# laomao0/BIN

Hardware: AMD Instinct MI355X
Metric: interpolated frames/sec at 1280x720 (higher is better)
Workload: dtype f16x3 (fp16 hi+lo pairs = 22-bit significands, 3 MFMA products, f32 accumulate; fp32-class: 1e-6 vs the fp32 reference); 1 GPU; Adobe240 test_blur 1280x720 inference, batch=1 per GPU (6-frame window padded to 768x1344 by the test.py rule), window-sharded; precision=f16x3, streams=1, pipelined_steps=False, four_call_schedule=False, parity=max-abs <= 2e-5 (f16x3) vs the fp32 reference (tests/)

## Files before the change

### bin_amd/_lib.py

```python
import ctypes as C
import os

from .build import GRAD_LIB_PATH, LIB_PATH, OPT_LIB_PATH

RDN_LAYERS = 66
RDN_MAX_LAYERS, RDN_MAX_CONVS = 192, 7
PLAN_KEEP_ACTS, PLAN_NO_FUSE, PLAN_RDB3, PLAN_FUSED_UPNET, PLAN_FUSED_UPNET_TRAIN = 1, 2, 4, 8, 16
BWD_ACCUMULATE = 1
BWD_SAVED_X3 = 2
BWD_FUSED_UPNET = 4
EPI_PLANES, EPI_SHUFFLE, EPI_FINAL, EPI_FINAL_SUBPIX = 0, 1, 2, 4
PROF_WGRAD = 16
LOSS_CHARBONNIER, LOSS_L1_SUM, LOSS_L2_SUM = 0, 1, 2
RDN_LAYOUT_WORDS, RDN_BWD_LAYOUT_WORDS = 16, 24


class BinConvDesc(C.Structure):
    _fields_ = [("N", C.c_int32), ("H", C.c_int32), ("W", C.c_int32), ("ksize", C.c_int32),
                ("cin_chunks", C.c_int32), ("cout", C.c_int32), ("cout_pad", C.c_int32),
                ("nterms", C.c_int32), ("epilogue", C.c_int32), ("relu", C.c_int32),
                ("x_cpg", C.c_int32), ("x_group_stride", C.c_int64), ("n_images", C.c_int32),
                ("reserved", C.c_int32), ("status", C.c_void_p)]


LOSS_MAX_TERMS = 24
CONV_HALF_LAST_CHUNK = 1


class BinLossTerms(C.Structure):
    _fields_ = [("x", C.c_void_p * LOSS_MAX_TERMS), ("y", C.c_void_p * LOSS_MAX_TERMS), ("n_terms", C.c_int32)]


class BinLossGrads(C.Structure):
    _fields_ = [("out", C.c_void_p * LOSS_MAX_TERMS), ("term_a", C.c_int32 * LOSS_MAX_TERMS),
                ("term_b", C.c_int32 * LOSS_MAX_TERMS), ("sign_a", C.c_float * LOSS_MAX_TERMS),
                ("sign_b", C.c_float * LOSS_MAX_TERMS), ("n_out", C.c_int32)]


class BinRdnShape(C.Structure):
    _fields_ = [("G0", C.c_int32), ("D", C.c_int32), ("C", C.c_int32), ("G", C.c_int32)]

# ... 235 lines not shown
```

### bin_amd/csrc/binhip_conv.hip

```cpp
#include "binhip_conv_common.h"
#include <vector>
#include <cstdio>
#include <cstdlib>

template <int KS, int MT, int WM, int R, int WN, int KC, int NT, int NBUF, int EPI>
struct ConvCfg {
    static constexpr int PAD = KS / 2;
    static constexpr int COUTB = 32 * MT * WM;
    static constexpr int TH = R * WN;
    static constexpr int PH = TH + KS - 1;
    static constexpr int PW = 32 + KS - 1;
    static constexpr int PP = (PH * PW * 2 + 63) / 64;
    static constexpr int WP = KS * KS * MT * WM;
    static constexpr int CHUNK_BYTES = (PP + WP) * 1024;
    static constexpr int NPL = (NT == 3) ? 2 : 1;
    static constexpr int PLANE_BYTES = KC * CHUNK_BYTES;
    static constexpr int BUF_BYTES = NPL * PLANE_BYTES;
    static constexpr int NW = WM * WN;
    static constexpr int LDS_BYTES = NBUF * BUF_BYTES + 1024;
    static constexpr int NPJ = (PP + NW - 1) / NW;
    static constexpr int NWJ = (WP + NW - 1) / NW;
    static constexpr int PS = NPL * KC * (NPJ + NWJ);
    static_assert(NW == 4 || NW == 8 || NW == 16, "4, 8 or 16 waves per workgroup");
    static_assert(LDS_BYTES <= 160 * 1024, "LDS budget");
// ... 229 lines not shown
    if (ksize == 3 && nterms == 3) return 32;
    if (ksize == 3 && cout_pad == 256) return 128;
    if (ksize == 5) return 32;
    if (ksize == 1 && cout_pad == 224) return 224;
    if (ksize == 1 && cout_pad == 1152) return 192;
    if (cout_pad % 96 == 0) return 96;
    if (ksize == 3 && cout_pad % 64 == 0) return 64;
    return 32;
}

static int bh_dispatch_conv(const ConvKArgs& a, int k, int cp, int nt, int e, hipStream_t s);
int bh_launch_conv_x3(const ConvKArgs& a, int cout_pad, int epilogue, hipStream_t s);
int bh_launch_final_dot2(const ConvKArgs& a, hipStream_t s);
int bh_launch_conv_x3_k5(const ConvKArgs& a, int cout_pad, hipStream_t s);
int bh_launch_conv_x3_k5_subpix(const ConvKArgs& a, hipStream_t s);
int bh_launch_final_m16(const ConvKArgs& a, hipStream_t s);

int bh_prepare_conv(const BhConvCall& c, ConvKArgs* out) {
    const BinConvDesc& d = c.d;
    if (!c.x_hi || !c.w_hi || !c.bias) return BINHIP_E_ARG;
    if (d.nterms != 1 && d.nterms != 3) return BINHIP_E_ARG;
    if (d.nterms == 3 && (!c.x_lo || !c.w_lo)) return BINHIP_E_ARG;
    if (d.N <= 0 || d.H <= 0 || d.W <= 0 || d.cin_chunks <= 0) return BINHIP_E_SHAPE;
    if ((long long)d.N * d.H * d.W >= (1ll << 26)) return BINHIP_E_SHAPE;
    ConvKArgs a;
    a.x_hi = (const _Float16*)c.x_hi; a.x_lo = (const _Float16*)c.x_lo;
    a.w_hi = (const _Float16*)c.w_hi; a.w_lo = (const _Float16*)c.w_lo;
    a.bias = c.bias;
    a.y_hi = (_Float16*)c.y_hi; a.y_lo = (_Float16*)c.y_lo;
    a.r_hi = (const _Float16*)c.r_hi; a.r_lo = (const _Float16*)c.r_lo;
    a.r2_hi = (const _Float16*)c.r2_hi; a.r2_lo = (const _Float16*)c.r2_lo;
    a.m_hi = (const _Float16*)c.m_hi;
    a.flags = (unsigned*)c.status;
    a.res_chunks = c.res_chunks > 0 ? c.res_chunks : (1 << 30);
    a.mask_from = c.mask_from;
    a.y_cpg = c.y_cpg; a.y_group_stride = c.y_group_stride;
    a.y_cpg_inv = c.y_cpg > 0 ? (unsigned)(((1u << 20) + c.y_cpg - 1) / c.y_cpg) : 0u;
    if (c.y_cpg > 128 || (c.y_cpg > 0 && d.cout_pad / 16 >= 4096)) return BINHIP_E_SHAPE;
    a.half_last = (d.reserved & BINHIP_CONV_HALF_LAST_CHUNK) ? 1 : 0;
    a.y_unshuf = c.y_unshuf;
    if (c.y_unshuf && (d.epilogue != BINHIP_EPI_PLANES || c.y_cpg > 0 || (d.H & 1) || (d.W & 1) || c.y_unshuf * 16 < d.cout))
        return BINHIP_E_SHAPE;
    if (c.r2_hi && d.nterms == 3 && !c.r2_lo) return BINHIP_E_ARG;
    a.out_f32 = c.y_f32;
    for (int i = 0; i < 5; ++i) a.img[i] = c.images[i];
    a.group_stride = d.x_group_stride;
    a.N = d.N; a.H = d.H; a.W = d.W;
    a.nchunks = d.cin_chunks;
    a.cpg = d.x_cpg;
    a.relu = d.relu; a.has_res = (c.r_hi != nullptr); a.nimg = d.n_images; a.cout = d.cout;
    a.och_limit = (d.epilogue == BINHIP_EPI_PLANES) ? (d.cout + 15) / 16 : (1 << 30);
    a.tiles_x = a.tiles_y = 0;
    a.ncol = 1;
    a.xcd_remap = 1;
    a.dbg = 0;
// ... 44 lines not shown
    const BinConvDesc& d = c.d;
    const int k = d.ksize, cp = d.cout_pad, nt = d.nterms, e = d.epilogue;
    if (bh_prof_begin(c.prof, k, cp, e, s)) {
        const int rc = bh_dispatch_conv(a, k, cp, nt, e, s);
        bh_prof_end(c.prof, s);
        return rc;
    }
    return bh_dispatch_conv(a, k, cp, nt, e, s);
}

static int bh_dispatch_conv(const ConvKArgs& a, int k, int cp, int nt, int e, hipStream_t s) {
    const int P = BINHIP_EPI_PLANES, S = BINHIP_EPI_SHUFFLE, F = BINHIP_EPI_FINAL;
    const int cb = bh_conv_cout_block(k, cp, nt);
    if (cb <= 0 || cp % cb) return BINHIP_E_SHAPE;
    if (e == BINHIP_EPI_FINAL_SUBPIX)
        return nt == 3 ? bh_launch_conv_x3_k5_subpix(a, s) : launch_cfg<5, 1, 1, 2, 8, 1, 1, 2, BINHIP_EPI_FINAL_SUBPIX>(a, cp, s);
    if (e == F && k == 3 && cp == 32 && a.cout <= 3 && nt == 1)
        return bh_launch_final_dot2(a, s);
    if (e == F && k == 3 && cp == 32 && a.cout <= 3 && nt == 3 && a.nchunks <= 4)
        return bh_launch_final_m16(a, s);
    if (nt == 1) {
        if (e == F && k == 3 && cp == 32) return launch_cfg<3, 1, 1, 2, 8, 1, 1, 2, F>(a, cp, s);
        if (e == S && k == 3 && cp == 256) return launch_cfg<3, 2, 2, 4, 4, 1, 1, 2, S>(a, cp, s);
        if (e == P && k == 3 && cb == 32)  return launch_cfg<3, 1, 1, 2, 8, 1, 1, 2, P>(a, cp, s);
        if (e == P && k == 3 && cb == 64)  return launch_cfg<3, 2, 1, 2, 4, 1, 1, 2, P>(a, cp, s);
        if (e == P && k == 3 && cb == 96)  return launch_cfg<3, 3, 1, 2, 4, 1, 1, 2, P>(a, cp, s);
        if (e == P && k == 3 && cb == 128) return launch_cfg<3, 2, 2, 4, 4, 1, 1, 2, P>(a, cp, s);
        if (e == P && k == 1 && cb == 224) return launch_cfg<1, 7, 1, 1, 8, 2, 1, 2, P>(a, cp, s);
        if (e == P && k == 1 && cb == 192) return launch_cfg<1, 6, 1, 1, 8, 2, 1, 2, P>(a, cp, s);
        if (e == P && k == 1 && cb == 32)  return launch_cfg<1, 1, 1, 4, 4, 4, 1, 2, P>(a, cp, s);
        if (e == P && k == 1 && cb == 96) {
// ... 346 lines not shown
    if (shuffle_perm && (cout % 4 || cout != cout_pad)) return BINHIP_E_SHAPE;
    const long long total = (long long)cout_pad * cin_chunks * ksize * ksize * 2;
    const int th = 256;
    const long long nb = (total + th - 1) / th;
    hipLaunchKernelGGL(relayout_kernel, dim3((unsigned)nb), dim3(th), 0, (hipStream_t)stream, w_oihw, bias, cout, cin,
                       ksize, cout_pad, cin_chunks, cout_block, shuffle_perm, (_Float16*)w_hi, (_Float16*)w_lo,
                       bias_out);
    BH_CHECK_LAUNCH();
    return 0;
}

int binhip_conv2d_fwd(const BinConvDesc* d, const void* x_hi, const void* x_lo, const void* w_hi,
                      const void* w_lo, const float* bias, const void* res_hi, const void* res_lo,
                      void* y_hi, void* y_lo, float* y_f32, const float* const* images, void* stream) {
    if (!d) return BINHIP_E_ARG;
    if (d->reserved & ~BINHIP_CONV_HALF_LAST_CHUNK) return BINHIP_E_ARG;
    if ((d->reserved & BINHIP_CONV_HALF_LAST_CHUNK) && d->ksize != 5) return BINHIP_E_ARG;
    BhConvCall c;
    c.d = *d;
    c.x_hi = x_hi; c.x_lo = x_lo; c.w_hi = w_hi; c.w_lo = w_lo; c.bias = bias;
    c.r_hi = res_hi; c.r_lo = res_lo; c.y_hi = y_hi; c.y_lo = y_lo; c.y_f32 = y_f32;
    c.status = d->status;
    for (int i = 0; i < 5; ++i) c.images[i] = (images && i < d->n_images) ? images[i] : nullptr;
    if (d->epilogue == BINHIP_EPI_FINAL && d->n_images > 0 && !images) return BINHIP_E_ARG;
    return bh_launch_conv(c, (hipStream_t)stream);
}

}
```

### bin_amd/csrc/binhip_conv_common.h

```cpp
#pragma once
#include "binhip_internal.h"
#ifndef BINHIP_TIMELINE
#define BINHIP_TIMELINE 0
#endif

typedef _Float16 half8 __attribute__((ext_vector_type(8)));
typedef _Float16 half4 __attribute__((ext_vector_type(4)));
typedef float floatx16 __attribute__((ext_vector_type(16)));
typedef float floatx4 __attribute__((ext_vector_type(4)));
typedef __attribute__((address_space(3))) void lds_void_t;
typedef unsigned u32x4 __attribute__((ext_vector_type(4)));

int bh_launch_upnet_ring(const void* x_hi, const void* x_lo, const float* wvar, const float* bvar, float* out, const float* const* images,
                         int nimg, int N, int H, int W, int cin, hipStream_t s);
int bh_upnet_gsub(const float* g, int N, int H, int W, const float* scale, void* y_hi, void* y_lo, void* status, hipStream_t s);
int bh_upnet_ring_dgrad(const float* g, const float* wvar, const float* scale, void* gx_hi, void* gx_lo, void* status, int N, int H, int W,
                        int cin, hipStream_t s);
int bh_upnet_ring_wgrad(const float* g, const void* x_hi, const void* x_lo, float* dwvar, float* dbvar, int N, int H, int W, int cin,
                        int accumulate, hipStream_t s);
struct ConvKArgs {
    const _Float16* x_hi;
    const _Float16* x_lo;
    const _Float16* w_hi;
    const _Float16* w_lo;
// ... 19 lines not shown
    int wt;
    int och_limit;
    int dbg;
    int res_chunks;
    int mask_from;
    int y_cpg;
    unsigned y_cpg_inv;
    long long y_group_stride;
    int prog_prio;
    int half_last;
#if BINHIP_TIMELINE
    void* tl;
    unsigned tl_launch;
    unsigned tl_base;
#endif
    int y_unshuf;
};

#if BINHIP_TIMELINE
#include <atomic>
struct BhTlRec {
    unsigned kind_launch, bid, hwid, xcc;
    unsigned long long rt[5];
    unsigned long long clk[2];
    unsigned long long pad;
};
static_assert(sizeof(BhTlRec) == 80, "record size (tools/wg_timeline.py)");
struct BhTlBuf { unsigned cursor, cap, pad[2]; BhTlRec rec[1]; };
inline void* g_bh_tl_buf = nullptr;
inline unsigned g_bh_tl_cap = 0;
// ... 30 lines not shown
        }
    }
};
#define BH_TL_DECL BhTl tl__
#define BH_TL_BEGIN() tl__.begin()
#define BH_TL_STAMP(i) tl__.stamp(i)
#define BH_TL_FINISH(a, i) tl__.finish((a).tl, (a).tl_launch, (a).tl_base + (unsigned)(i))
#else
#define BH_TL_DECL
#define BH_TL_BEGIN()
#define BH_TL_STAMP(i)
#define BH_TL_FINISH(a, i)
#endif

#define BINHIP_EPI_PLANES_LFFD 3

template <int N>
__device__ __forceinline__ void wait_vmcnt() {
    asm volatile("s_waitcnt vmcnt(%0)" ::"n"(N) : "memory");
}

__device__ __forceinline__ void store16(_Float16* base, long long off_elems, uint4 v, int wt) {
    if (wt) {
        __amdgpu_buffer_rsrc_t rs = __builtin_amdgcn_make_buffer_rsrc((void*)base, 0, 0xFFFFFFFFu, 0x00020000);
        u32x4 d = {v.x, v.y, v.z, v.w};
        __builtin_amdgcn_raw_buffer_store_b128(d, rs, (int)(off_elems * 2), 0, 16);
    } else {
        *reinterpret_cast<uint4*>(base + off_elems) = v;
    }
}
// ... 4 lines not shown
}

template <int MT, int R, int NT, int EPI, bool XTRA>
__device__ __forceinline__ void conv_epilogue(const ConvKArgs& a, const float* __restrict__ bias, floatx16 (&acc)[MT][R],
                                              int img, int row0, int tx0, int co0, bool first_col, int n, int kg,
                                              long long plane_elems) {
    const int H = a.H, W = a.W;
    const int gx = tx0 + n;
    auto bias4 = [&](int co_u, float (&bv)[4]) {
        float b8[8];
#pragma unroll
        for (int j = 0; j < 8; ++j) b8[j] = bias[co_u + j];
#pragma unroll
        for (int j = 0; j < 4; ++j) bv[j] = kg ? b8[4 + j] : b8[j];
    };
    if constexpr (EPI == BINHIP_EPI_FINAL_SUBPIX) {
        const int ncolour = a.cout >> 2;
        const int H2 = 2 * H, W2 = 2 * W;
        float bv[2][4];
        bias4(co0, bv[0]);
        bias4(co0 + 8, bv[1]);
        const bool col_ok = first_col && (gx < W);
        float sum[R][2][4];
#pragma unroll
        for (int r = 0; r < R; ++r) {
            const int gy = row0 + r;
#pragma unroll
            for (int g = 0; g < 2; ++g) {
                const int c = 2 * g + kg;
                const bool ok = col_ok && gy < H && c < ncolour;
#pragma unroll
                for (int q = 0; q < 4; ++q) {
                    float sj = 0.f;
                    if (ok && a.nimg > 0) {
                        const long long idx = (((long long)img * ncolour + c) * H2 + 2 * gy + (q >> 1)) * W2 + 2 * gx + (q & 1);
                        sj = a.img[0][idx];
                        for (int t = 1; t < a.nimg; ++t) sj += a.img[t][idx];
                        sj = sj / (float)a.nimg;
                    }
                    sum[r][g][q] = sj;
                }
            }
        }
#pragma unroll
        for (int r = 0; r < R; ++r) {
            const int gy = row0 + r;
#pragma unroll
            for (int g = 0; g < 2; ++g) {
                const int c = 2 * g + kg;
                if (!(col_ok && gy < H && c < ncolour)) continue;
#pragma unroll
                for (int q = 0; q < 4; ++q) {
                    const long long idx = (((long long)img * ncolour + c) * H2 + 2 * gy + (q >> 1)) * W2 + 2 * gx + (q & 1);
                    a.out_f32[idx] = (acc[0][r][4 * g + q] + bv[g][q]) + sum[r][g][q];
                }
            }
        }
    } else if constexpr (EPI == BINHIP_EPI_FINAL) {
        float bv[4];
        bias4(co0, bv);
        const bool mine = (kg == 0) && first_col && (gx < W);
        float sum[R][4];
#pragma unroll
        for (int r = 0; r < R; ++r) {
// ... 269 lines not shown
```

### bin_amd/csrc/binhip_conv_x3.hip

```cpp
#include "binhip_conv_common.h"
constexpr int X3_R = 2, X3_WN = 8;

template <int KS, int R, int WN>
struct X3Cfg {
    static constexpr int PAD = KS / 2;
    static constexpr int TH = R * WN;
    static constexpr int PH = TH + KS - 1;
    static constexpr int PW = 32 + KS - 1;
    static constexpr int PP = (PH * PW * 2 + 63) / 64;
    static constexpr int WP = KS * KS;
    static constexpr int NW = WN;
    static constexpr int PATCH_BYTES = PP * 1024;
    static constexpr int WBUF_BYTES = 2 * WP * 1024;
    static constexpr int LDS_BYTES = 2 * PATCH_BYTES + 2 * WBUF_BYTES;
    static constexpr int NPJ = (PP + NW - 1) / NW;
    static constexpr int NWJ = (2 * WP + NW - 1) / NW;
    static_assert((KS == 3 ? 2 : 1) * LDS_BYTES <= 160 * 1024, "LDS budget");
};

template <class C>
__device__ __forceinline__ void x3_issue_patch(const ConvKArgs& a, char* smem, int c, int pl, int buf, int wave,
                                               const unsigned* voff, long long plane_elems, unsigned plane_bytes) {
    const _Float16* xb = pl ? a.x_lo : a.x_hi;
    const long long coff = (a.cpg > 0) ? (long long)(c / a.cpg) * a.group_stride + (long long)(c % a.cpg) * plane_elems
// ... 674 lines not shown
    a.tiles_y = (a.H + C::TH - 1) / C::TH;
    a.ncol = 1;
    dim3 grid((unsigned)(a.tiles_x * a.tiles_y * a.N));
    const unsigned* wh = reinterpret_cast<const unsigned*>(a.w_hi);
    final_dot2_kernel<1><<<grid, dim3(256), 2 * C::PATCH_BYTES, s>>>(a, wh, wh);
    BH_CHECK_LAUNCH();
    return 0;
}

int bh_launch_conv_x3_k5(const ConvKArgs& a, int cout_pad, hipStream_t s) {
    return launch_x3<5, X3_R, X3_WN, BINHIP_EPI_PLANES, 1>(a, cout_pad, s);
}

int bh_launch_conv_x3_k5_subpix(const ConvKArgs& a, hipStream_t s) {
    return launch_x3<5, X3_R, X3_WN, BINHIP_EPI_FINAL_SUBPIX, 0>(a, 32, s);
}

struct RingArgs {
    const _Float16* x_hi;
    const _Float16* x_lo;
    const float* wvar;
    const float* bvar;
    float* out;
    const float* img[5];
    int N, H, W, cin, nimg;
};
constexpr int RING_THREADS = 128;
__global__ void __launch_bounds__(RING_THREADS) upnet_ring_kernel(const RingArgs a) {
    __shared__ float red[3][RING_THREADS / 64];
    const int tid = threadIdx.x, lane = tid & 63, wave = tid >> 6;
// ... 83 lines not shown
```

### bin_amd/csrc/binhip_plan.hip

```cpp
#include "binhip_conv_common.h"

namespace {

struct Shp {
    int G0, D, C, G;
    int c0, cg, cb;
    int L;
    bool stage4;
};
bool resolve_shape(const BinRdnShape* s, Shp* o) {
    Shp h;
    const bool dflt = !s || (s->G0 == 0 && s->D == 0 && s->C == 0 && s->G == 0);
    h.G0 = dflt ? 96 : s->G0; h.D = dflt ? 12 : s->D; h.C = dflt ? 4 : s->C; h.G = dflt ? 32 : s->G;
    if (h.G0 < 32 || h.G0 > 256 || h.G0 % 32 || h.G < 32 || h.G > 128 || h.G % 32) return false;
    if (h.C < 1 || h.C > BINHIP_RDN_MAX_CONVS || h.D < 1 || h.D > 20) return false;
    h.c0 = h.G0 / 16; h.cg = h.G / 16; h.cb = h.c0 + h.C * h.cg;
    h.L = 2 + h.D * (h.C + 1) + 4;
    if (h.L > BINHIP_RDN_MAX_LAYERS) return false;
    h.stage4 = (h.G0 == 96 && h.C == 4 && h.G == 32);
    *o = h;
    return true;
}
inline int layer_conv(const Shp& sh, int d, int c) { return 2 + d * (sh.C + 1) + c; }

// ... 152 lines not shown
            if ((rc = binhip_rdb_tail_fwd(N, h, ww, nt, HI(b), LO(b, w.s_blk), p->w_hi[L3], p->w_lo[L3], p->bias[L3],
                                          p->w_hi[LF], p->w_lo[LF], p->bias[LF], HI(b + (int64_t)cb * P),
                                          LO(b + (int64_t)cb * P, w.s_blk), (p->reserved & BINHIP_PLAN_KEEP_ACTS) ? 1 : 0, p->status, stream)))
                return rc;
        } else if ((rc = conv(layer_conv(sh, d, C), 1, cb, G0, G0, P_, 0, h, ww, b, w.s_blk, 0, 0, b + (int64_t)cb * P, w.s_blk, b, w.s_blk)))
            return rc;
    }
    const int LG = sh.L - 4;
    if ((rc = conv(LG, 1, D * c0, G0, G0, P_, 0, h, ww, w.blk + (int64_t)cb * P, w.s_blk, c0, (int64_t)cb * P, w.g0, w.s_g, -1, 0))) return rc;
    if ((rc = conv(LG + 1, 3, c0, G0, G0, P_, 0, h, ww, w.g0, w.s_g, 0, 0, w.g1, w.s_g, w.f1, w.s_f1))) return rc;
    const bool fused_up = (p->reserved & BINHIP_PLAN_FUSED_UPNET) &&
                          (!(p->reserved & BINHIP_PLAN_KEEP_ACTS) || (p->reserved & BINHIP_PLAN_FUSED_UPNET_TRAIN)) &&
                          sh.L + 1 < BINHIP_RDN_MAX_LAYERS && p->w_hi[sh.L] && (nt == 1 || p->w_lo[sh.L]) && p->bias[sh.L] &&
                          p->w_hi[sh.L + 1] && p->bias[sh.L + 1];
    if (fused_up) {
        if ((rc = bh_launch_conv(mk(sh.L, 5, c0, 12, 32, BINHIP_EPI_FINAL_SUBPIX, 0, h, ww, w.g1, w.s_g, 0, 0, -1, 0, -1, 0), s))) return rc;
        return bh_launch_upnet_ring(HI(w.g1), LO(w.g1, w.s_g), (const float*)p->w_hi[sh.L + 1], p->bias[sh.L + 1], out, inputs, nin, N, h, ww,
                                    G0, s);
    }
    if ((rc = conv(LG + 2, 3, c0, 256, 256, BINHIP_EPI_SHUFFLE, 0, h, ww, w.g1, w.s_g, 0, 0, w.u, w.s_u, -1, 0))) return rc;
    if ((rc = conv(LG + 3, 3, 4, 3, 32, BINHIP_EPI_FINAL, 0, H, W, w.u, w.s_u, 0, 0, -1, 0, -1, 0))) return rc;
    return 0;
}

}

namespace {

struct Bws {
    int64_t P, PF;
    int kc0, gx0_chunks;
// ... 247 lines not shown
```

### bin_amd/ops.py

```python
import ctypes as C
import os

import torch

from . import _lib as L


def _stream(device=None):
    return C.c_void_p(torch.cuda.current_stream(device).cuda_stream)


def on_device(t):
    return torch.cuda.device(t.device)


_status = {}


def status_word(device):
    key = _device_key(device)
    w = _status.get(key)
    if w is None:
        w = torch.zeros(1, dtype=torch.int32, device=torch.device("cuda", key))
        _status[key] = w
# ... 147 lines not shown
                                            self.cout_block, 1 if shuffle else 0, _ptr(self.w_hi), _ptr(self.w_lo),
                                            _ptr(self.bias), _stream()), "weights_relayout")


def conv2d(x, cw, relu=False, residual=None, out=None, epilogue=L.EPI_PLANES, images=None, x_cpg=0,
           x_group_stride=0, cin_chunks=None):
    nch, n, h, w, _ = x.hi.shape
    d = L.BinConvDesc()
    d.N, d.H, d.W, d.ksize = n, h, w, cw.ks
    d.cin_chunks = cin_chunks if cin_chunks is not None else cw.cin_chunks
    d.cout, d.cout_pad, d.nterms, d.epilogue, d.relu = cw.cout, cw.cout_pad, cw.nterms, epilogue, int(relu)
    d.x_cpg, d.x_group_stride = x_cpg, x_group_stride
    d.n_images = len(images) if images else 0
    if cw.ks == 5 and 1 <= cw.cin % 16 <= 8 and d.cin_chunks == cw.cin_chunks:
        d.reserved = L.CONV_HALF_LAST_CHUNK
    dev = x.hi.device
    d.status = status_word(dev).data_ptr()
    y_f32, arr = None, None
    if epilogue == L.EPI_PLANES:
        if out is None:
            out = CP.empty(chunks(cw.cout), n, h, w, cw.nterms, dev, cw.cout)
    elif epilogue == L.EPI_SHUFFLE:
        if out is None:
            out = CP.empty(chunks(cw.cout // 4), n, 2 * h, 2 * w, cw.nterms, dev, cw.cout // 4)
    else:
        y_f32 = torch.empty((n, cw.cout, h, w), dtype=torch.float32, device=dev)
        if images:
            images = [im.contiguous().float() for im in images]
            arr = (C.c_void_p * len(images))(*[im.data_ptr() for im in images])
    rc = L.lib().binhip_conv2d_fwd(
        C.byref(d), _ptr(x.hi), _ptr(x.lo), _ptr(cw.w_hi), _ptr(cw.w_lo), _ptr(cw.bias),
        _ptr(residual.hi) if residual is not None else C.c_void_p(0),
        _ptr(residual.lo) if residual is not None else C.c_void_p(0),
        _ptr(out.hi) if out is not None else C.c_void_p(0),
        _ptr(out.lo) if out is not None else C.c_void_p(0),
        _ptr(y_f32), arr, _stream())
    L.check(rc, "conv2d_fwd")
    return y_f32 if epilogue == L.EPI_FINAL else out


def convlstm_cell(x, state, weight, bias, forget_bias=1.0):
    _need_cuda(x, weight)
    x = x.contiguous().float()
    n, c, h, w = x.shape
    assert c == 3 and tuple(weight.shape) == (12, 6, 3, 3)
    cn = torch.empty_like(x)
    hn = torch.empty_like(x)
    cp = state[0].contiguous().float() if state is not None else None
    hp = state[1].contiguous().float() if state is not None else None
    L.check(L.lib().binhip_convlstm_fwd(_ptr(x), _ptr(cp), _ptr(hp), _ptr(weight.detach().contiguous().float()),
                                        _ptr(bias.detach().contiguous().float()), float(forget_bias), n, h, w,
                                        _ptr(cn), _ptr(hn), _stream()), "convlstm_fwd")
    return hn, [cn, hn]
# ... 514 lines not shown
```

### bin_amd/rdn_plan.py

```python
import ctypes as C

import torch

from . import _lib as L
from .ops import ConvWeights, _ptr, _stream, _need_cuda, on_device, relayout_batch, relayout_item, status_word

STAGE4_SHAPE = (96, 12, 4, 32)


def check_shape(shape):
    G0, D, C, G = (int(v) for v in shape)
    if G0 % 32 or not 32 <= G0 <= 256 or G % 32 or not 32 <= G <= 128 or not 1 <= C <= L.RDN_MAX_CONVS or not 1 <= D <= 20 \
            or 2 + D * (C + 1) + 4 > L.RDN_MAX_LAYERS:
        raise NotImplementedError(
            f"bin_amd RDN: unsupported configuration G0={G0}, D={D}, C={C}, G={G} (built: G0 and G multiples of 32 with "
            f"32 <= G0 <= 256, G <= 128; 1 <= C <= {L.RDN_MAX_CONVS}; 1 <= D <= 20)")
    return G0, D, C, G


def c_shape(shape):
    s = L.BinRdnShape()
    s.G0, s.D, s.C, s.G = shape
    return s

# ... 124 lines not shown
    import torch.nn.functional as F
    x = x.double()
    out = F.pixel_shuffle(F.conv2d(x, W[4], B[4], padding=2), 2)
    h2, w2 = out.shape[-2:]
    for vy in range(3):
        for vx in range(3):
            if vy == 1 and vx == 1:
                continue
            full = F.pixel_shuffle(F.conv2d(x, W[3 * vy + vx], B[3 * vy + vx], padding=2), 2)
            ys = {0: slice(0, 1), 1: slice(1, h2 - 1), 2: slice(h2 - 1, h2)}[vy]
            xs = {0: slice(0, 1), 1: slice(1, w2 - 1), 2: slice(w2 - 1, w2)}[vx]
            out[..., ys, xs] = full[..., ys, xs]
    return out


class RdnWeights:

    def __init__(self, params, n_inputs, nterms, prefix="", shape=STAGE4_SHAPE):
        self.n_inputs, self.nterms, self.shape = n_inputs, nterms, check_shape(shape)
        self.layers = []
        items = []
        for i, nm in enumerate(layer_names(self.shape)):
            w, b = params[f"{prefix}{nm}.weight"], params[f"{prefix}{nm}.bias"]
            shuffle = nm == "UPNet.0"
            cin_chunks = None
            if nm == "SFENet1":
                cin_chunks = (12 * n_inputs + 15) // 16
            self.layers.append(ConvWeights(w, b, nterms=nterms, shuffle=shuffle, cin_chunks=cin_chunks, defer=items))
        assert len(self.layers) == 2 + self.shape[1] * (self.shape[2] + 1) + 4
        relayout_batch(items)

        self._dgrad = None
        w0, _, w2, _ = src = tuple(params[f"{prefix}UPNet.{k}.{t}"] for k in (0, 2) for t in ("weight", "bias"))
        fusable = tuple(w0.shape[2:]) == (3, 3) and w0.shape[0] == 256 and tuple(w2.shape) == (3, 64, 3, 3)
        self._up_src = src if fusable else None
        self.fused_up = None
        self.fused_w4 = None
        self.fused_train = None
        self.fused_train_w4 = None
        self.fused_graph = None

    def ensure_fused_upnet(self, train=False):
        if self._up_src is None:
            return None
        if train:
            if self.fused_train is None:
                with torch.enable_grad():
                    leaves = [t.detach().float().requires_grad_() for t in self._up_src]
                    Wr, Br = fused_upnet_operator(*leaves)
                self.fused_graph = (leaves, Wr, Br)
                with torch.no_grad():
                    g0 = Wr.shape[3]
                    self.fused_train_w4 = Wr[4].permute(0, 2, 1).reshape(12, g0, 5, 5).contiguous()
                    main = ConvWeights(self.fused_train_w4, Br[4].detach().contiguous(), nterms=self.nterms)
                    self.fused_train = (main, Wr.detach().contiguous(), Br.detach().contiguous())
            return self.fused_train
        if self.fused_up is None:
            with torch.no_grad():
                W, B = fused_upnet_weights(*self._up_src)
                self.fused_w4 = W[4].float().contiguous()
                main = ConvWeights(self.fused_w4, B[4].float().contiguous(), nterms=self.nterms)
                ring_w = W.permute(0, 1, 3, 4, 2).reshape(9, 12, 25, W.shape[2]).float().contiguous()
                self.fused_up = (main, ring_w, B.float().contiguous())
        return self.fused_up

    def fill_plan(self, plan, fused=None):
        plan.shape = c_shape(self.shape)
        for i, cw in enumerate(self.layers):
            plan.w_hi[i] = cw.w_hi.data_ptr()
            plan.w_lo[i] = cw.w_lo.data_ptr() if cw.w_lo is not None else None
            plan.bias[i] = cw.bias.data_ptr()
        n = len(self.layers)
        if fused is not None:
            main, ring_w, ring_b = fused
            plan.w_hi[n], plan.bias[n] = main.w_hi.data_ptr(), main.bias.data_ptr()
            plan.w_lo[n] = main.w_lo.data_ptr() if main.w_lo is not None else None
            plan.w_hi[n + 1], plan.w_lo[n + 1], plan.bias[n + 1] = ring_w.data_ptr(), None, ring_b.data_ptr()

    def dgrad(self, module, nterms=None, fused=False):
        nterms = self.nterms if nterms is None else nterms
        if self._dgrad is None:
            self._dgrad = {}
        key = (nterms, bool(fused))
        if key not in self._dgrad:
            if fused and self.fused_train is None:
                raise RuntimeError("bin_amd: backward of a fused-UPNet forward on weights that never built the training operands")
            with torch.no_grad():
                self._dgrad[key] = RdnDgradWeights(dict(module.named_parameters()), self.n_inputs, nterms, shape=self.shape,
                                                   fused=(self.fused_train_w4, self.fused_train[1]) if fused else None)
        return self._dgrad[key]


# ... 85 lines not shown
def release_workspaces(stream=None):
    if stream is None:
        _workspaces.clear()
        return
    for k in [k for k in _workspaces if k[2] == stream.cuda_stream and k[1] == stream.device.index]:
        del _workspaces[k]


import os as _os


def default_plan_flags():
    flags = L.PLAN_RDB3 if _os.environ.get("BIN_AMD_RDB3", "0") == "1" else 0
    if _os.environ.get("BIN_AMD_FUSED_UPNET", "1") != "0":
        flags |= L.PLAN_FUSED_UPNET
    return flags


def rdn_forward(weights, inputs, out=None, ws=None, flags=0, profiler=None):
    _need_cuda(*inputs)
    with on_device(inputs[0]):
        return _rdn_forward(weights, inputs, out, ws, flags, profiler)


def _rdn_forward(weights, inputs, out, ws, flags, profiler):
    inputs = [t.contiguous().float() for t in inputs]
    n, c, h, w = inputs[0].shape
    assert c == 3 and len(inputs) == weights.n_inputs
    lib = L.lib()
    plan = L.BinRdnPlan()
    plan.N, plan.H, plan.W, plan.n_inputs, plan.nterms = n, h, w, weights.n_inputs, weights.nterms
    plan.reserved = int(flags or 0)
    plan.status = status_word(inputs[0].device).data_ptr()
    plan.profiler = profiler if profiler else None
    fused = None
    if plan.reserved & L.PLAN_FUSED_UPNET:
        if plan.reserved & L.PLAN_FUSED_UPNET_TRAIN:
            fused = weights.ensure_fused_upnet(train=True)
        elif not (plan.reserved & L.PLAN_KEEP_ACTS):
            fused = weights.ensure_fused_upnet()
    weights.fill_plan(plan, fused)
    nbytes = lib.binhip_rdn_workspace_bytes(n, h, w, weights.n_inputs, weights.nterms, C.byref(plan.shape))
    if nbytes == 0:
        raise RuntimeError(f"bin_amd: unsupported RDN shape N={n} H={h} W={w} (H, W must be even)")
    if ws is None:
        ws = workspace(nbytes, inputs[0].device)
    if out is None:
        out = torch.empty((n, 3, h, w), dtype=torch.float32, device=inputs[0].device)
    arr = (C.c_void_p * len(inputs))(*[t.data_ptr() for t in inputs])
    L.check(lib.binhip_rdn_forward(C.byref(plan), arr, _ptr(out), _ptr(ws), ws.numel(), _stream()), "rdn_forward")
    return out
```

### include/binhip.h

```cpp
#ifndef BINHIP_H
#define BINHIP_H

#include <stddef.h>
#include <stdint.h>

#ifdef __cplusplus
extern "C" {
#endif

#define BINHIP_API __attribute__((visibility("default")))

#define BINHIP_VERSION 622
#define BINHIP_ABI_EXPORTS 51

#define BINHIP_E_ARG      (-1)
#define BINHIP_E_SHAPE    (-2)
#define BINHIP_E_WORKSPACE (-3)

#define BINHIP_STATUS_SATURATED 1u
#define BINHIP_STATUS_SYNC_TIMEOUT 2u

#define BINHIP_EPI_PLANES  0
#define BINHIP_EPI_SHUFFLE 1
#define BINHIP_EPI_FINAL   2
// ... 13 lines not shown
    int32_t ksize;
    int32_t cin_chunks;
    int32_t cout;
    int32_t cout_pad;
    int32_t nterms;
    int32_t epilogue;
    int32_t relu;
    int32_t x_cpg;
    int64_t x_group_stride;
    int32_t n_images;
    int32_t reserved;
    void*   status;
} BinConvDesc;

#define BINHIP_CONV_HALF_LAST_CHUNK 1

BINHIP_API int binhip_conv_cout_block(int ksize, int cout_pad, int nterms);

BINHIP_API int binhip_weights_relayout(const float* w_oihw, const float* bias, int cout, int cin, int ksize,
                            int cout_pad, int cin_chunks, int cout_block, int shuffle_perm,
                            void* w_hi, void* w_lo, float* bias_out, void* stream);
BINHIP_API size_t binhip_weights_bytes(int cout_pad, int cin_chunks, int ksize);
#define BINHIP_RELAYOUT_FWD        0
#define BINHIP_RELAYOUT_DGRAD      1
#define BINHIP_RELAYOUT_RDB_GATHER 2
typedef struct BinRelayoutItem {
    const float* w[BINHIP_RDN_MAX_CONVS + 1];
    const float* bias;
    void* w_hi;
    void* w_lo;
// ... 75 lines not shown
    int32_t n_out;
} BinLossGrads;
BINHIP_API int binhip_multi_loss_bwd(int kind, const BinLossTerms* t, int64_t numel, float eps, const float* gloss,
                          const BinLossGrads* g, void* stream);

BINHIP_API int binhip_rdb_tail_fwd(int N, int H, int W, int nterms, const void* blk_hi, const void* blk_lo,
                        const void* wc_hi, const void* wc_lo, const float* bias_c,
                        const void* wl_hi, const void* wl_lo, const float* bias_l,
                        void* y_hi, void* y_lo, int store_o3, void* status, void* stream);

#define BINHIP_PLAN_KEEP_ACTS 1
#define BINHIP_PLAN_NO_FUSE   2
#define BINHIP_PLAN_RDB3      4
#define BINHIP_PLAN_FUSED_UPNET 8
#define BINHIP_PLAN_FUSED_UPNET_TRAIN 16
typedef struct BinRdnPlan {
    int32_t N, H, W;
    int32_t n_inputs;
    int32_t nterms;
    int32_t reserved;
    BinRdnShape shape;
    const void* w_hi[BINHIP_RDN_MAX_LAYERS];
    const void* w_lo[BINHIP_RDN_MAX_LAYERS];
    const float* bias[BINHIP_RDN_MAX_LAYERS];
    void* status;
    struct BinhipProfiler* profiler;
} BinRdnPlan;

BINHIP_API size_t binhip_rdn_workspace_bytes(int N, int H, int W, int n_inputs, int nterms, const BinRdnShape* shape );
#define BINHIP_RDN_LAYOUT_WORDS 16
// ... 82 lines not shown
```

Measured before the change: 15.67 interpolated frames/s.

## Fold two output rows into padded MFMA M dimension for upnet 5x5 subpixel conv

The upnet 5x5 conv has only 12 real output channels but is padded to a 32-row MFMA tile, so most of the tile is wasted. This adds a folded weight layout that stacks two vertically shifted copies of the 12-channel filter (6x5 taps) into rows 0-11 and 12-23, and a dedicated kernel that computes two output rows per accumulator. The epilogue is adapted to map folded rows back to colour and row. The aim is to cut MFMA and weight traffic per output pixel, at the cost of a 6x5 instead of 5x5 tap loop, a new kernel, and extra host-side weight preparation. It is enabled by default through an environment flag.

```diff
diff --git a/bin_amd/_lib.py b/bin_amd/_lib.py
--- a/bin_amd/_lib.py
+++ b/bin_amd/_lib.py
@@ -5,7 +5,7 @@
 
 RDN_LAYERS = 66
 RDN_MAX_LAYERS, RDN_MAX_CONVS = 192, 7
-PLAN_KEEP_ACTS, PLAN_NO_FUSE, PLAN_RDB3, PLAN_FUSED_UPNET, PLAN_FUSED_UPNET_TRAIN = 1, 2, 4, 8, 16
+PLAN_KEEP_ACTS, PLAN_NO_FUSE, PLAN_RDB3, PLAN_FUSED_UPNET, PLAN_FUSED_UPNET_TRAIN, PLAN_UPNET_FOLD = 1, 2, 4, 8, 16, 32
 BWD_ACCUMULATE = 1
 BWD_SAVED_X3 = 2
 BWD_FUSED_UPNET = 4
@@ -25,6 +25,7 @@
 
 LOSS_MAX_TERMS = 24
 CONV_HALF_LAST_CHUNK = 1
+CONV_UPNET_FOLD = 2
 
 
 class BinLossTerms(C.Structure):
diff --git a/bin_amd/csrc/binhip_conv.hip b/bin_amd/csrc/binhip_conv.hip
--- a/bin_amd/csrc/binhip_conv.hip
+++ b/bin_amd/csrc/binhip_conv.hip
@@ -267,6 +267,7 @@
 int bh_launch_final_dot2(const ConvKArgs& a, hipStream_t s);
 int bh_launch_conv_x3_k5(const ConvKArgs& a, int cout_pad, hipStream_t s);
 int bh_launch_conv_x3_k5_subpix(const ConvKArgs& a, hipStream_t s);
+int bh_launch_conv_x3_k5_subpix_fold(const ConvKArgs& a, hipStream_t s);
 int bh_launch_final_m16(const ConvKArgs& a, hipStream_t s);
 
 int bh_prepare_conv(const BhConvCall& c, ConvKArgs* out) {
@@ -292,6 +293,8 @@
     if (c.y_cpg > 128 || (c.y_cpg > 0 && d.cout_pad / 16 >= 4096)) return BINHIP_E_SHAPE;
     a.half_last = (d.reserved & BINHIP_CONV_HALF_LAST_CHUNK) ? 1 : 0;
     a.y_unshuf = c.y_unshuf;
+    a.up_fold = (d.reserved & BINHIP_CONV_UPNET_FOLD) ? 1 : 0;
+    if (a.up_fold && (d.epilogue != BINHIP_EPI_FINAL_SUBPIX || d.nterms != 3 || d.cout != 12)) return BINHIP_E_ARG;
     if (c.y_unshuf && (d.epilogue != BINHIP_EPI_PLANES || c.y_cpg > 0 || (d.H & 1) || (d.W & 1) || c.y_unshuf * 16 < d.cout))
         return BINHIP_E_SHAPE;
     if (c.r2_hi && d.nterms == 3 && !c.r2_lo) return BINHIP_E_ARG;
@@ -366,7 +369,8 @@
     const int cb = bh_conv_cout_block(k, cp, nt);
     if (cb <= 0 || cp % cb) return BINHIP_E_SHAPE;
     if (e == BINHIP_EPI_FINAL_SUBPIX)
-        return nt == 3 ? bh_launch_conv_x3_k5_subpix(a, s) : launch_cfg<5, 1, 1, 2, 8, 1, 1, 2, BINHIP_EPI_FINAL_SUBPIX>(a, cp, s);
+        return nt == 3 ? (a.up_fold ? bh_launch_conv_x3_k5_subpix_fold(a, s) : bh_launch_conv_x3_k5_subpix(a, s))
+                       : launch_cfg<5, 1, 1, 2, 8, 1, 1, 2, BINHIP_EPI_FINAL_SUBPIX>(a, cp, s);
     if (e == F && k == 3 && cp == 32 && a.cout <= 3 && nt == 1)
         return bh_launch_final_dot2(a, s);
     if (e == F && k == 3 && cp == 32 && a.cout <= 3 && nt == 3 && a.nchunks <= 4)
@@ -743,7 +747,7 @@
                       const void* w_lo, const float* bias, const void* res_hi, const void* res_lo,
                       void* y_hi, void* y_lo, float* y_f32, const float* const* images, void* stream) {
     if (!d) return BINHIP_E_ARG;
-    if (d->reserved & ~BINHIP_CONV_HALF_LAST_CHUNK) return BINHIP_E_ARG;
+    if (d->reserved & ~(BINHIP_CONV_HALF_LAST_CHUNK | BINHIP_CONV_UPNET_FOLD)) return BINHIP_E_ARG;
     if ((d->reserved & BINHIP_CONV_HALF_LAST_CHUNK) && d->ksize != 5) return BINHIP_E_ARG;
     BhConvCall c;
     c.d = *d;
diff --git a/bin_amd/csrc/binhip_conv_common.h b/bin_amd/csrc/binhip_conv_common.h
--- a/bin_amd/csrc/binhip_conv_common.h
+++ b/bin_amd/csrc/binhip_conv_common.h
@@ -57,6 +57,7 @@
     unsigned tl_launch;
     unsigned tl_base;
 #endif
+    int up_fold;
     int y_unshuf;
 };
 
@@ -117,6 +118,7 @@
 #endif
 
 #define BINHIP_EPI_PLANES_LFFD 3
+#define BINHIP_EPI_FINAL_SUBPIX_FOLD 5
 
 template <int N>
 __device__ __forceinline__ void wait_vmcnt() {
@@ -151,20 +153,24 @@
 #pragma unroll
         for (int j = 0; j < 4; ++j) bv[j] = kg ? b8[4 + j] : b8[j];
     };
-    if constexpr (EPI == BINHIP_EPI_FINAL_SUBPIX) {
+    if constexpr (EPI == BINHIP_EPI_FINAL_SUBPIX || EPI == BINHIP_EPI_FINAL_SUBPIX_FOLD) {
+        constexpr bool FOLD = EPI == BINHIP_EPI_FINAL_SUBPIX_FOLD;
+        static_assert(!FOLD || (MT == 1 && R == 1), "one folded accumulator");
+        constexpr int NG = FOLD ? 3 : 2;
         const int ncolour = a.cout >> 2;
         const int H2 = 2 * H, W2 = 2 * W;
-        float bv[2][4];
-        bias4(co0, bv[0]);
-        bias4(co0 + 8, bv[1]);
+        float bv[NG][4];
+#pragma unroll
+        for (int g = 0; g < NG; ++g) bias4(co0 + 8 * g, bv[g]);
         const bool col_ok = first_col && (gx < W);
-        float sum[R][2][4];
+        float sum[R][NG][4];
 #pragma unroll
         for (int r = 0; r < R; ++r) {
-            const int gy = row0 + r;
-#pragma unroll
-            for (int g = 0; g < 2; ++g) {
-                const int c = 2 * g + kg;
+#pragma unroll
+            for (int g = 0; g < NG; ++g) {
+                const int m = 2 * g + kg;
+                const int c = FOLD ? m % 3 : m;
+                const int gy = row0 + (FOLD ? m / 3 : r);
                 const bool ok = col_ok && gy < H && c < ncolour;
 #pragma unroll
                 for (int q = 0; q < 4; ++q) {
@@ -181,10 +187,11 @@
         }
 #pragma unroll
         for (int r = 0; r < R; ++r) {
-            const int gy = row0 + r;
-#pragma unroll
-            for (int g = 0; g < 2; ++g) {
-                const int c = 2 * g + kg;
+#pragma unroll
+            for (int g = 0; g < NG; ++g) {
+                const int m = 2 * g + kg;
+                const int c = FOLD ? m % 3 : m;
+                const int gy = row0 + (FOLD ? m / 3 : r);
                 if (!(col_ok && gy < H && c < ncolour)) continue;
 #pragma unroll
                 for (int q = 0; q < 4; ++q) {
diff --git a/bin_amd/csrc/binhip_conv_x3.hip b/bin_amd/csrc/binhip_conv_x3.hip
--- a/bin_amd/csrc/binhip_conv_x3.hip
+++ b/bin_amd/csrc/binhip_conv_x3.hip
@@ -712,6 +712,141 @@
 
 int bh_launch_conv_x3_k5_subpix(const ConvKArgs& a, hipStream_t s) {
     return launch_x3<5, X3_R, X3_WN, BINHIP_EPI_FINAL_SUBPIX, 0>(a, 32, s);
+}
+
+struct UpFold {
+    using C = X3Cfg<5, X3_R, X3_WN>;
+    static constexpr int NSTEP = 6 * 5;
+    static constexpr int W_BYTES = NSTEP * 1024;
+    static constexpr int WHI_OFF = 2 * C::PATCH_BYTES;
+    static constexpr int WLO_OFF = WHI_OFF + 2 * W_BYTES;
+    static constexpr int LDS_BYTES = WLO_OFF + W_BYTES;
+    static constexpr int NWJ = (NSTEP + C::NW - 1) / C::NW;
+    static_assert(LDS_BYTES <= 160 * 1024, "LDS budget: one workgroup per CU");
+};
+
+__device__ __forceinline__ void upfold_issue_weights(const _Float16* plane, char* dst, int c, int wave, int lane) {
+    __amdgpu_buffer_rsrc_t rs =
+        __builtin_amdgcn_make_buffer_rsrc((void*)(plane + (long long)c * (UpFold::NSTEP * 32 * 16)), 0, UpFold::W_BYTES, 0x00020000);
+#pragma unroll
+    for (int j = 0; j < UpFold::NWJ; ++j) {
+        const int i = wave + UpFold::C::NW * j;
+        if (i < UpFold::NSTEP)
+            __builtin_amdgcn_raw_ptr_buffer_load_lds(rs, (lds_void_t*)(dst + i * 1024), 16, (unsigned)(lane * 16), i * 1024, 0, 0);
+    }
+}
+
+template <bool HI>
+__device__ __forceinline__ void upfold_compute(const char* pb, const char* wh, const char* wl, int a_lane_off, int b_lane_off,
+                                               floatx16& acc) {
+    using C = UpFold::C;
+    constexpr int NI = 6, NS = UpFold::NSTEP;
+    half8 B[2][NI];
+    half8 Ah[2], Al[2];
+    auto load_b = [&](int dx, half8 (&dst)[NI]) {
+#pragma unroll
+        for (int i = 0; i < NI; ++i) dst[i] = x3_ld8(pb + b_lane_off + (i * C::PW + dx) * 16);
+    };
+    auto load_a = [&](int s, half8& h, half8& l) {
+        const int dx = s / NI, i = s % NI;
+        const int off = (i * 5 + dx) * 1024 + a_lane_off;
+        h = x3_ld8(wh + off);
+        if constexpr (HI) l = x3_ld8(wl + off);
+    };
+    load_b(0, B[0]);
+    load_a(0, Ah[0], Al[0]);
+#pragma unroll
+    for (int s = 0; s < NS; ++s) {
+        const int dx = s / NI, i = s % NI;
+        if (s + 1 < NS) load_a(s + 1, Ah[(s + 1) & 1], Al[(s + 1) & 1]);
+        if (i == 0 && dx + 1 < 5) load_b(dx + 1, B[(dx + 1) & 1]);
+        __builtin_amdgcn_sched_barrier(0);
+        if constexpr (HI) acc = x3_mfma(Al[s & 1], B[dx & 1][i], acc);
+        acc = x3_mfma(Ah[s & 1], B[dx & 1][i], acc);
+        __builtin_amdgcn_sched_barrier(0);
+    }
+}
+
+__global__ void __launch_bounds__(64 * X3_WN) __attribute__((amdgpu_waves_per_eu(X3_WN / 4, X3_WN / 4)))
+conv_x3_upfold_kernel(const ConvKArgs a, const float* __restrict__ bias) {
+    using C = UpFold::C;
+    extern __shared__ __attribute__((aligned(16))) char smem[];
+    int bid = blockIdx.x;
+    if (a.xcd_remap) bid = xcd_band(bid, gridDim.x);
+    const int tx = bid % a.tiles_x;
+    bid /= a.tiles_x;
+    const int ty = bid % a.tiles_y;
+    const int img = bid / a.tiles_y;
+    const int tid = threadIdx.x;
+    const int lane = tid & 63;
+    const int wave = __builtin_amdgcn_readfirstlane(tid >> 6);
+    const int n = lane & 31;
+    const int kg = lane >> 5;
+    const int tx0 = tx * 32, ty0 = ty * C::TH;
+    const int H = a.H, W = a.W;
+    const long long plane_elems = (long long)a.N * H * W * 16;
+    const unsigned plane_bytes = (unsigned)(plane_elems * 2);
+
+    unsigned voff[C::NPJ];
+#pragma unroll
+    for (int j = 0; j < C::NPJ; ++j) {
+        const int i = wave + C::NW * j;
+        const int q = i * 64 + lane;
+        const int cg = q >= C::PH * C::PW ? 1 : 0;
+        const int p = q - cg * (C::PH * C::PW);
+        const int py = p / C::PW;
+        const int px = p - py * C::PW;
+        const int gy = ty0 + py - C::PAD;
+        const int gx = tx0 + px - C::PAD;
+        const bool ok = (p < C::PH * C::PW) && (gy >= 0) && (gy < H) && (gx >= 0) && (gx < W);
+        voff[j] = ok ? (unsigned)((((long long)img * H + gy) * W + gx) * 32 + cg * 16) : 0x80000000u;
+    }
+    floatx16 acc[1][1];
+#pragma unroll
+    for (int e = 0; e < 16; ++e) acc[0][0][e] = 0.f;
+
+    const int nchunks = a.nchunks;
+    const int a_lane_off = n * 32 + ((kg ^ ((n >> 3) & 1)) << 4);
+    const int b_lane_off = (kg * (C::PH * C::PW) + wave * X3_R * C::PW + n) * 16;
+    char* const wlo = smem + UpFold::WLO_OFF;
+
+    __builtin_amdgcn_s_setprio(2);
+    upfold_issue_weights(a.w_hi, smem + UpFold::WHI_OFF, 0, wave, lane);
+    upfold_issue_weights(a.w_lo, wlo, 0, wave, lane);
+    x3_issue_patch<C>(a, smem, 0, 0, 0, wave, voff, plane_elems, plane_bytes);
+    for (int c = 0; c < nchunks; ++c) {
+        const char* whi = smem + UpFold::WHI_OFF + (c & 1) * UpFold::W_BYTES;
+        wait_vmcnt<0>();
+        __builtin_amdgcn_s_barrier();
+        __builtin_amdgcn_sched_barrier(0);
+        x3_issue_patch<C>(a, smem, c, 1, 1, wave, voff, plane_elems, plane_bytes);
+        if (c + 1 < nchunks) upfold_issue_weights(a.w_hi, smem + UpFold::WHI_OFF + ((c + 1) & 1) * UpFold::W_BYTES, c + 1, wave, lane);
+        upfold_compute<true>(smem, whi, wlo, a_lane_off, b_lane_off, acc[0][0]);
+        wait_vmcnt<0>();
+        __builtin_amdgcn_s_barrier();
+        __builtin_amdgcn_sched_barrier(0);
+        if (c + 1 < nchunks) {
+            x3_issue_patch<C>(a, smem, c + 1, 0, 0, wave, voff, plane_elems, plane_bytes);
+            upfold_issue_weights(a.w_lo, wlo, c + 1, wave, lane);
+        }
+        upfold_compute<false>(smem + C::PATCH_BYTES, whi, wlo, a_lane_off, b_lane_off, acc[0][0]);
+    }
+    __builtin_amdgcn_s_setprio(0);
+    conv_epilogue<1, 1, 3, BINHIP_EPI_FINAL_SUBPIX_FOLD, false>(a, bias, acc, img, ty0 + wave * X3_R, tx0, 0, true, n, kg, plane_elems);
+}
+
+int bh_launch_conv_x3_k5_subpix_fold(const ConvKArgs& ka, hipStream_t s) {
+    using C = UpFold::C;
+    static std::atomic<unsigned long long> lds_set{0};
+    if (ka.cout != 12) return BINHIP_E_SHAPE;
+    if (int rc = bh_set_max_lds(&conv_x3_upfold_kernel, UpFold::LDS_BYTES, lds_set)) return rc;
+    ConvKArgs a = ka;
+    a.tiles_x = (a.W + 31) / 32;
+    a.tiles_y = (a.H + C::TH - 1) / C::TH;
+    a.ncol = 1;
+    conv_x3_upfold_kernel<<<dim3((unsigned)(a.tiles_x * a.tiles_y * a.N)), dim3(64 * C::NW), UpFold::LDS_BYTES, s>>>(a, a.bias);
+    BH_CHECK_LAUNCH();
+    return 0;
 }
 
 struct RingArgs {
diff --git a/bin_amd/csrc/binhip_plan.hip b/bin_amd/csrc/binhip_plan.hip
--- a/bin_amd/csrc/binhip_plan.hip
+++ b/bin_amd/csrc/binhip_plan.hip
@@ -190,7 +190,11 @@
                           sh.L + 1 < BINHIP_RDN_MAX_LAYERS && p->w_hi[sh.L] && (nt == 1 || p->w_lo[sh.L]) && p->bias[sh.L] &&
                           p->w_hi[sh.L + 1] && p->bias[sh.L + 1];
     if (fused_up) {
-        if ((rc = bh_launch_conv(mk(sh.L, 5, c0, 12, 32, BINHIP_EPI_FINAL_SUBPIX, 0, h, ww, w.g1, w.s_g, 0, 0, -1, 0, -1, 0), s))) return rc;
+        const bool fold = (p->reserved & BINHIP_PLAN_UPNET_FOLD) && nt == 3 && !(p->reserved & BINHIP_PLAN_KEEP_ACTS) &&
+                          sh.L + 2 < BINHIP_RDN_MAX_LAYERS && p->w_hi[sh.L + 2] && p->w_lo[sh.L + 2] && p->bias[sh.L + 2];
+        BhConvCall up = mk(fold ? sh.L + 2 : sh.L, 5, c0, 12, 32, BINHIP_EPI_FINAL_SUBPIX, 0, h, ww, w.g1, w.s_g, 0, 0, -1, 0, -1, 0);
+        if (fold) up.d.reserved = BINHIP_CONV_UPNET_FOLD;
+        if ((rc = bh_launch_conv(up, s))) return rc;
         return bh_launch_upnet_ring(HI(w.g1), LO(w.g1, w.s_g), (const float*)p->w_hi[sh.L + 1], p->bias[sh.L + 1], out, inputs, nin, N, h, ww,
                                     G0, s);
     }
diff --git a/bin_amd/ops.py b/bin_amd/ops.py
--- a/bin_amd/ops.py
+++ b/bin_amd/ops.py
@@ -185,6 +185,8 @@
     d.n_images = len(images) if images else 0
     if cw.ks == 5 and 1 <= cw.cin % 16 <= 8 and d.cin_chunks == cw.cin_chunks:
         d.reserved = L.CONV_HALF_LAST_CHUNK
+    if getattr(cw, "fold", False):
+        d.reserved |= L.CONV_UPNET_FOLD
     dev = x.hi.device
     d.status = status_word(dev).data_ptr()
     y_f32, arr = None, None
@@ -195,7 +197,8 @@
         if out is None:
             out = CP.empty(chunks(cw.cout // 4), n, 2 * h, 2 * w, cw.nterms, dev, cw.cout // 4)
     else:
-        y_f32 = torch.empty((n, cw.cout, h, w), dtype=torch.float32, device=dev)
+        shape = (n, cw.cout // 4, 2 * h, 2 * w) if epilogue == L.EPI_FINAL_SUBPIX else (n, cw.cout, h, w)
+        y_f32 = torch.empty(shape, dtype=torch.float32, device=dev)
         if images:
             images = [im.contiguous().float() for im in images]
             arr = (C.c_void_p * len(images))(*[im.data_ptr() for im in images])
@@ -207,7 +210,7 @@
         _ptr(out.lo) if out is not None else C.c_void_p(0),
         _ptr(y_f32), arr, _stream())
     L.check(rc, "conv2d_fwd")
-    return y_f32 if epilogue == L.EPI_FINAL else out
+    return y_f32 if epilogue in (L.EPI_FINAL, L.EPI_FINAL_SUBPIX) else out
 
 
 def convlstm_cell(x, state, weight, bias, forget_bias=1.0):
diff --git a/bin_amd/rdn_plan.py b/bin_amd/rdn_plan.py
--- a/bin_amd/rdn_plan.py
+++ b/bin_amd/rdn_plan.py
@@ -162,6 +162,38 @@
     return out
 
 
+def fold_upnet_operator(w):
+    assert w.shape[0] == 12 and tuple(w.shape[2:]) == (5, 5)
+    f = w.new_zeros(32, w.shape[1], 6, 5)
+    f[0:12, :, 0:5] = w
+    f[12:24, :, 1:6] = w
+    return f
+
+
+def fold_upnet_slab(slab, cin_chunks):
+    s = slab.view(cin_chunks, 5, 5, 32, 2, 8)
+    f = s.new_zeros(cin_chunks, 6, 5, 32, 2, 8)
+    f[:, 0:5, :, 0:12] = s[:, :, :, 0:12]
+    low = s[:, :, :, 0:12]
+    swap = [m for m in range(12) if ((m >> 3) & 1) != (((12 + m) >> 3) & 1)]
+    low = low.clone()
+    low[:, :, :, swap] = low[:, :, :, swap].flip(-2)
+    f[:, 1:6, :, 12:24] = low
+    return f.reshape(-1)
+
+
+class FoldedUpnetWeights:
+    fold = True
+
+    def __init__(self, main):
+        assert main.ks == 5 and main.cout == 12 and main.cout_pad == 32 and main.nterms == 3
+        self.cout, self.cin, self.ks, self.nterms, self.shuffle = 12, main.cin, 5, 3, False
+        self.cout_pad, self.cin_chunks, self.cout_block = 32, main.cin_chunks, main.cout_block
+        self.w_hi = fold_upnet_slab(main.w_hi, main.cin_chunks)
+        self.w_lo = fold_upnet_slab(main.w_lo, main.cin_chunks)
+        self.bias = torch.cat((main.bias[:12], main.bias[:12], main.bias.new_zeros(8))).contiguous()
+
+
 class RdnWeights:
 
     def __init__(self, params, n_inputs, nterms, prefix="", shape=STAGE4_SHAPE):
@@ -183,6 +215,7 @@
         fusable = tuple(w0.shape[2:]) == (3, 3) and w0.shape[0] == 256 and tuple(w2.shape) == (3, 64, 3, 3)
         self._up_src = src if fusable else None
         self.fused_up = None
+        self.fused_fold = None
         self.fused_w4 = None
         self.fused_train = None
         self.fused_train_w4 = None
@@ -209,10 +242,11 @@
                 self.fused_w4 = W[4].float().contiguous()
                 main = ConvWeights(self.fused_w4, B[4].float().contiguous(), nterms=self.nterms)
                 ring_w = W.permute(0, 1, 3, 4, 2).reshape(9, 12, 25, W.shape[2]).float().contiguous()
+                self.fused_fold = FoldedUpnetWeights(main) if self.nterms == 3 else None
                 self.fused_up = (main, ring_w, B.float().contiguous())
         return self.fused_up
 
-    def fill_plan(self, plan, fused=None):
+    def fill_plan(self, plan, fused=None, fold=None):
         plan.shape = c_shape(self.shape)
         for i, cw in enumerate(self.layers):
             plan.w_hi[i] = cw.w_hi.data_ptr()
@@ -224,6 +258,8 @@
             plan.w_hi[n], plan.bias[n] = main.w_hi.data_ptr(), main.bias.data_ptr()
             plan.w_lo[n] = main.w_lo.data_ptr() if main.w_lo is not None else None
             plan.w_hi[n + 1], plan.w_lo[n + 1], plan.bias[n + 1] = ring_w.data_ptr(), None, ring_b.data_ptr()
+            if fold is not None:
+                plan.w_hi[n + 2], plan.w_lo[n + 2], plan.bias[n + 2] = fold.w_hi.data_ptr(), fold.w_lo.data_ptr(), fold.bias.data_ptr()
 
     def dgrad(self, module, nterms=None, fused=False):
         nterms = self.nterms if nterms is None else nterms
@@ -339,6 +375,8 @@
     flags = L.PLAN_RDB3 if _os.environ.get("BIN_AMD_RDB3", "0") == "1" else 0
     if _os.environ.get("BIN_AMD_FUSED_UPNET", "1") != "0":
         flags |= L.PLAN_FUSED_UPNET
+    if _os.environ.get("BIN_AMD_UPNET_FOLD", "1") != "0":
+        flags |= L.PLAN_UPNET_FOLD
     return flags
 
 
@@ -358,13 +396,15 @@
     plan.reserved = int(flags or 0)
     plan.status = status_word(inputs[0].device).data_ptr()
     plan.profiler = profiler if profiler else None
-    fused = None
+    fused = fold = None
     if plan.reserved & L.PLAN_FUSED_UPNET:
         if plan.reserved & L.PLAN_FUSED_UPNET_TRAIN:
             fused = weights.ensure_fused_upnet(train=True)
         elif not (plan.reserved & L.PLAN_KEEP_ACTS):
             fused = weights.ensure_fused_upnet()
-    weights.fill_plan(plan, fused)
+            if fused is not None and (plan.reserved & L.PLAN_UPNET_FOLD):
+                fold = weights.fused_fold
+    weights.fill_plan(plan, fused, fold)
     nbytes = lib.binhip_rdn_workspace_bytes(n, h, w, weights.n_inputs, weights.nterms, C.byref(plan.shape))
     if nbytes == 0:
         raise RuntimeError(f"bin_amd: unsupported RDN shape N={n} H={h} W={w} (H, W must be even)")
diff --git a/include/binhip.h b/include/binhip.h
--- a/include/binhip.h
+++ b/include/binhip.h
@@ -51,6 +51,7 @@
 } BinConvDesc;
 
 #define BINHIP_CONV_HALF_LAST_CHUNK 1
+#define BINHIP_CONV_UPNET_FOLD 2
 
 BINHIP_API int binhip_conv_cout_block(int ksize, int cout_pad, int nterms);
 
@@ -156,6 +157,7 @@
 #define BINHIP_PLAN_RDB3      4
 #define BINHIP_PLAN_FUSED_UPNET 8
 #define BINHIP_PLAN_FUSED_UPNET_TRAIN 16
+#define BINHIP_PLAN_UPNET_FOLD 32
 typedef struct BinRdnPlan {
     int32_t N, H, W;
     int32_t n_inputs;
```

Measured after the change: 15.82 interpolated frames/s, median of 6. No clear change (+1.0%).
